# aleflabo/COSKAD

Hardware: AMD Instinct MI355X
Metric: pose_clips_per_sec_fwd_bwd (higher is better)
Workload: dtype f32; 1 GPU; euclidean_encoder_dynamicCenter train step (fwd+mse-to-centre+L2 reg+bwd+Adam), synthetic clips B=4096/GPU T=12 V=17 C=2, channels 2-32-16-32-64, latent 16; clips_per_gpu=4096, global_batch=4096, head=euclidean, parallelism=dp1, hip_graph=False

## Files before the change

### coskad_amd/csrc/fused_apply_bpc.hip

```cpp
#include "fused_ops.h"
#include "layer_launch.h"

namespace coskad {
namespace fpc {

using namespace ff;

#ifndef BPC_GRID
#define BPC_GRID (256 * BPC_OCC)
#endif
#ifndef BPC_OCC
#define BPC_OCC 3
#endif
template <int CT>
__global__ __launch_bounds__(256, BPC_OCC) void k_layer_apply_bpc(const float* __restrict__ in, const float* __restrict__ Zg,
                                                           const float* __restrict__ wfold, const float* __restrict__ bias,
                                                           const float* __restrict__ in_slope, float* __restrict__ out, int B) {
  constexpr int Ci = 16 * CT, Co = 64, CoP = Co, NG = 2 * CT;
  extern __shared__ __attribute__((aligned(16))) float lds[];
  float* r1 = lds;
  float* r2 = lds + 32 * LD;
  const int tid = threadIdx.x, lane = tid & 63;
  const int wave = __builtin_amdgcn_readfirstlane(tid >> 6);
  auto geo = [&]() {
    int l = lane;
    asm volatile("" : "+v"(l));
    return Lane{l & 15, l >> 4};
  };
  Lane L = geo();
  const bool pre = in_slope != nullptr;
  const float a_in = pre ? in_slope[0] : 0.f;
  const BufRes wres = make_res(wfold, 2 * Ci * CoP * 4u);
  const BufRes bres = make_res(bias, CoP * 4u);
  auto clip_res = [&](const float* base, int c, int rows) {
    const bool in_range = c < B;
#ifdef COSKAD_HOT
    return make_res(base + (size_t)(in_range ? (c & 63) : 0) * rows * TV, in_range ? rows * TV * 4u : 0u);
#else
    return make_res(base + (size_t)(in_range ? c : 0) * rows * TV, in_range ? rows * TV * 4u : 0u);
#endif
  };
  constexpr int Q4 = 4 * (TV / 4);
  const bool stg = tid < Q4;
  const int srow = tid / (TV / 4), scol = 4 * (tid - srow * (TV / 4));
  const int svoff = stg ? tid * 16 : 0x7ffffff0;
#ifndef BPC_DEPTH
#define BPC_DEPTH 2
#endif
  constexpr int DEPTH = BPC_DEPTH;
  float4 gq[DEPTH][4];
  auto qload = [&](const BufRes& res, int row0, int q) { return buf_load4(res, svoff, (row0 + 4 * q) * (TV / 4) * 16); };
  auto qstore = [&](int q, float4 v, bool act) {
    if (act) { v.x = prelu(v.x, a_in); v.y = prelu(v.y, a_in); v.z = prelu(v.z, a_in); v.w = prelu(v.w, a_in); }
    if (stg) *reinterpret_cast<float4*>(r2 + (4 * q + srow) * LDW + scol) = v;
  };

  int clip = blockIdx.x;
  {
    const BufRes z0 = clip_res(Zg, clip, Ci), x0 = clip_res(in, clip, Ci);
#pragma unroll
    for (int q = 0; q < 4; ++q) {
      gq[0][q] = qload(z0, 0, q);
      if (DEPTH == 2) gq[DEPTH - 1][q] = CT > 1 ? qload(z0, 16, q) : qload(x0, 0, q);
    }
  }
  for (; clip < B; clip += gridDim.x) {
    const BufRes xres = clip_res(in, clip, Ci), zres = clip_res(Zg, clip, Ci), ores = clip_res(out, clip, Co);
    const BufRes znext = clip_res(Zg, clip + gridDim.x, Ci), xnext = clip_res(in, clip + gridDim.x, Ci);
    auto vload = [&](int vg, int q) {
      const bool nxt = vg >= NG;
      const int g = nxt ? vg - NG : vg;
      return g < CT ? qload(nxt ? znext : zres, 16 * g, q) : qload(nxt ? xnext : xres, 16 * (g - CT), q);
    };
    L = geo();
    const int jc = L.j < T ? L.j : T - 1;
    f32x4 acc[NTILE];
#pragma unroll
    for (int t = 0; t < NTILE; ++t) acc[t] = f32x4{0.f, 0.f, 0.f, 0.f};
#pragma unroll
    for (int q = 0; q < 4; ++q) {
      qstore(q, gq[0][q], false);
      gq[0][q] = vload(DEPTH, q);
    }
    const int lq = (L.q * CoP + 16 * wave + L.j) * 4;
    float wc[2][4];
#pragma unroll
    for (int s = 0; s < 4; ++s) wc[0][s] = buf_load1(wres, lq, (4 * s) * CoP * 4);
    __syncthreads();
#ifndef BPC_BDBL
#define BPC_BDBL 0
#endif
    float b[1 + BPC_BDBL][NTILE];
#pragma unroll
    for (int t = 0; t < NTILE; ++t) b[0][t] = r2[L.q * LDW + (t < T ? t * V + L.j : jc * V + 16)];
#pragma unroll
    for (int g = 0; g < NG; ++g) {
      if (g + 1 < NG) {
#pragma unroll
        for (int s = 0; s < 4; ++s) wc[(g + 1) & 1][s] = buf_load1(wres, lq, ((16 * (g + 1) + 4 * s) * CoP) * 4);
      }
#pragma unroll
      for (int s = 0; s < 4; ++s) {
        if (BPC_BDBL && (s + 1 < 4 || g + 1 < NG)) {
          const int sn = (s + 1) & 3;
#pragma unroll
          for (int t = 0; t < NTILE; ++t) b[(s + 1) & 1][t] = r2[(4 * sn + L.q) * LDW + (t < T ? t * V + L.j : jc * V + 16)];
        }
        if (g + 1 < NG || s == 0) __syncthreads();
        if (g + 1 < NG) {
          qstore(s, gq[(g + 1) % DEPTH][s], g + 1 >= CT && pre);
          if (DEPTH == 2 || g + 2 < NG) gq[(g + 1) % DEPTH][s] = vload(g + 1 + DEPTH, s);
        }
#pragma unroll
        for (int t = 0; t < NTILE; ++t) acc[t] = mfma(wc[g & 1][s], b[BPC_BDBL ? (s & 1) : 0][t], acc[t]);
        if (!BPC_BDBL && (s + 1 < 4 || g + 1 < NG)) {
          const int sn = (s + 1) & 3;
#pragma unroll
          for (int t = 0; t < NTILE; ++t) b[0][t] = r2[(4 * sn + L.q) * LDW + (t < T ? t * V + L.j : jc * V + 16)];
        }
      }
    }
    if (DEPTH == 1) {
#pragma unroll
      for (int q = 0; q < 4; ++q) gq[0][q] = vload(NG, q);
    }
    L = geo();
    const float4 b4 = buf_load4(bres, L.q * 16, (16 * wave) * 4);
    const f32x4 bq = {b4.x, b4.y, b4.z, b4.w};
    const int jf = L.j < T ? L.j : T - 1;
#pragma unroll
    for (int rnd = 0; rnd < 2; ++rnd) {
      if ((wave >> 1) == rnd) {
#pragma unroll
        for (int t = 0; t < NTILE; ++t)
          tile_store(r1, 16 * (wave & 1), t < T ? t * V + L.j : jf * V + 16, t < T || L.j < T, acc[t] + bq, L);
      }
      __syncthreads();
      constexpr int n4 = 32 * (TV / 4);
#pragma unroll
      for (int i = 0; i < (n4 + 255) / 256; ++i) {
        const int e4 = tid + 256 * i;
        const bool ok = e4 < n4;
        const int row = e4 / (TV / 4), col = 4 * (e4 - row * (TV / 4));
        const float* p = r1 + (ok ? row * LD + col : PADCOL);
        const float2 g0 = *reinterpret_cast<const float2*>(p), g1 = *reinterpret_cast<const float2*>(p + 2);
        buf_store4(ores, ok ? e4 * 16 : 0x7ffffff0, (32 * rnd) * (TV / 4) * 16, float4{g0.x, g0.y, g1.x, g1.y});
      }
      __syncthreads();
    }
  }
}

}

int launch_layer_apply_bpc(const float* Z, const float* in, float* out, const float* wfold, const float* bias,
                           const float* in_slope, int B, int Ci, int Co, hipStream_t st) {
  if (!(Ci == 32 && Co == 64)) return fail(COSKAD_ERR_SHAPE, "apply_bpc: built for 32 -> 64 channels (%d, %d)", Ci, Co);
  const size_t lds = (size_t)ff::WAVE_LDS_W * sizeof(float);
  const int grid = B < BPC_GRID ? B : BPC_GRID;
  auto k = fpc::k_layer_apply_bpc<2>;
  {
    ProbeScope probe(KID_LAYER_APPLY, Ci, Co, st);
    hipLaunchKernelGGL(k, dim3(grid), dim3(256), lds, st, in, Z, wfold, bias, in_slope, out, B);
  }
  return check_launch("layer_apply_bpc");
}

}
```

### coskad_amd/csrc/fused_apply_next_bpc.hip

```cpp
#include "fused_ops.h"
#include "layer_launch.h"

namespace coskad {
namespace fnb {

using namespace ff;

#ifndef FNB_OCC
#define FNB_OCC 4
#endif

template <int CT, int OTP>
__global__ __launch_bounds__(256, FNB_OCC) void k_layer_apply_next_bpc(const float* __restrict__ in, const float* __restrict__ Zg,
                                                                      const float* __restrict__ wfold, const float* __restrict__ bias,
                                                                      const float* __restrict__ in_slope,
                                                                      const float* __restrict__ out_slope,
                                                                      const float* __restrict__ ftab, float* __restrict__ out,
                                                                      float* __restrict__ Znext, float* __restrict__ partials, int B) {
  constexpr int Ci = CT ? 16 * CT : 2, Co = 16 * OTP, CoP = Co, NG = 2 * CT;
  constexpr int NACC = OTP == 1 ? 2 : 3;
  constexpr int E = 2 * (Co * Co + Co);
  constexpr int MAXT = OTP == 2 ? 7 : 4;
  extern __shared__ __attribute__((aligned(16))) float lds[];
  float* r1 = lds;
  float* r2 = lds + 32 * LD;
  const int tid = threadIdx.x, lane = tid & 63;
  const int wave = __builtin_amdgcn_readfirstlane(tid >> 6);
  auto geo = [&]() {
    int l = lane;
    asm volatile("" : "+v"(l));
    return Lane{l & 15, l >> 4};
  };
  auto olane = [&]() {
    int l = lane;
    asm volatile("" : "+v"(l));
    return l;
  };
  const bool pre = in_slope != nullptr;
  const float a_in = pre ? in_slope[0] : 0.f;
  const float a_out = out_slope[0];
  const int l16 = lane * 16;
  const BufRes wres = make_res(wfold, 2 * Ci * CoP * 4u);
  const BufRes bres = make_res(bias, CoP * 4u);
  const BufRes tabres = make_res(ftab, LAYER_F4 * 16u);
  auto clip_res = [&](const float* base, int c, int rows) {
    const bool in_range = c < B;
    return make_res(base + (size_t)(in_range ? c : 0) * rows * TV, in_range ? rows * TV * 4u : 0u);
  };
  const int ot = OTP == 2 ? (wave & 1) : 0;
  const int t0 = OTP == 2 ? ((wave >> 1) ? 7 : 0) : (wave == 0 ? 0 : 1 + 3 * wave);
  const int nt = OTP == 2 ? ((wave >> 1) ? 6 : 7) : (wave == 0 ? 4 : 3);
  constexpr int Q4 = 4 * (TV / 4);
  const bool stg = tid < Q4;
  const int srow = tid / (TV / 4), scol = 4 * (tid - srow * (TV / 4));
  const int svoff = stg ? tid * 16 : 0x7ffffff0;
  constexpr int DEPTH = CT == 1 ? 1 : 2;
  float4 gq[DEPTH][4];
  auto qload = [&](const BufRes& res, int row0, int q) { return buf_load4(res, svoff, (row0 + 4 * q) * (TV / 4) * 16); };
  auto qstore = [&](int q, float4 v, bool act) {
    if (act) { v.x = prelu(v.x, a_in); v.y = prelu(v.y, a_in); v.z = prelu(v.z, a_in); v.w = prelu(v.w, a_in); }
    if (stg) *reinterpret_cast<float4*>(r2 + (4 * q + srow) * LDW + scol) = v;
  };
  const bool fst = tid < 2 * (TV / 4);
  const int frow = tid / (TV / 4), fcol = 4 * (tid - frow * (TV / 4));
  const int fvoff = fst ? tid * 16 : 0x7ffffff0;

  f32x4 gx[NACC], gz[NACC];
  float sx[OTP], sz[OTP];
#pragma unroll
  for (int i = 0; i < NACC; ++i) { gx[i] = f32x4{0.f, 0.f, 0.f, 0.f}; gz[i] = f32x4{0.f, 0.f, 0.f, 0.f}; }
#pragma unroll
  for (int i = 0; i < OTP; ++i) { sx[i] = 0.f; sz[i] = 0.f; }
  auto gram_rows = [&](f32x4 (&g)[NACC], float (&s)[OTP], const BufRes& ores, bool act) {
    const Lane L = geo();
    const float* p0 = r1 + L.j * LD + 2 * L.q;
    const float* p1 = r1 + (16 + L.j) * LD + 2 * L.q;
    constexpr int NM = (TV + 7) / 8;
    constexpr int n4 = Co * (TV / 4), NI = (n4 + 63) / 64;
    const int ln = olane();
    for (int m = wave; m < NM; m += 4) {
      float2 a0 = *reinterpret_cast<const float2*>(p0 + 8 * m);
      float2 a1 = OTP == 2 ? *reinterpret_cast<const float2*>(p1 + 8 * m) : float2{0.f, 0.f};
      if (act) {
        a0.x = prelu(a0.x, a_out); a0.y = prelu(a0.y, a_out);
        a1.x = prelu(a1.x, a_out); a1.y = prelu(a1.y, a_out);
      }
      const bool ok = 8 * m + 2 * L.q < TV;
      a0.x = ok ? a0.x : 0.f; a0.y = ok ? a0.y : 0.f;
      a1.x = ok ? a1.x : 0.f; a1.y = ok ? a1.y : 0.f;
      if constexpr (OTP == 1) {
        g[0] = mfma(a0.x, a0.x, g[0]);
        g[1] = mfma(a0.y, a0.y, g[1]);
        s[0] += a0.x + a0.y;
      } else {
        g[0] = mfma(a0.x, a0.x, g[0]);
        g[1] = mfma(a0.x, a1.x, g[1]);
        g[2] = mfma(a1.x, a1.x, g[2]);
        g[0] = mfma(a0.y, a0.y, g[0]);
        g[1] = mfma(a0.y, a1.y, g[1]);
        g[2] = mfma(a1.y, a1.y, g[2]);
        s[0] += a0.x + a0.y;
        s[OTP - 1] += a1.x + a1.y;
      }
      const int i = OTP == 2 ? m : (m & 1 ? -1 : m >> 1);
      if (i >= 0 && i < NI) {
        const int e4 = ln + 64 * i;
        const int row = e4 / (TV / 4), col = 4 * (e4 - row * (TV / 4));
        const bool okp = e4 < n4;
        const float* ptr = r1 + (okp ? row * LD + col : PADCOL);
        const float2 g0 = *reinterpret_cast<const float2*>(ptr), g1 = *reinterpret_cast<const float2*>(ptr + 2);
        buf_store4(ores, okp ? e4 * 16 : 0x7ffffff0, 0, float4{g0.x, g0.y, g1.x, g1.y});
      }
    }
  };

  int clip = blockIdx.x;
  {
    const BufRes z0 = clip_res(Zg, clip, Ci), x0 = clip_res(in, clip, Ci);
    if (CT == 0) {
      gq[0][0] = buf_load4(z0, fvoff, 0);
      gq[0][1] = buf_load4(x0, fvoff, 0);
    } else {
#pragma unroll
      for (int q = 0; q < 4; ++q) {
        gq[0][q] = qload(z0, 0, q);
        if (DEPTH == 2) gq[DEPTH - 1][q] = qload(z0, 16, q);
      }
    }
  }
  for (; clip < B; clip += gridDim.x) {
    const BufRes xres = clip_res(in, clip, Ci), zres = clip_res(Zg, clip, Ci), ores = clip_res(out, clip, Co);
    const BufRes znext = clip_res(Zg, clip + gridDim.x, Ci), xnext = clip_res(in, clip + gridDim.x, Ci);
    const BufRes zores = clip_res(Znext, clip, Co);
    Lane L = geo();
    const int jc = L.j < T ? L.j : T - 1;
    f32x4 acc[MAXT];
#pragma unroll
    for (int t = 0; t < MAXT; ++t) acc[t] = f32x4{0.f, 0.f, 0.f, 0.f};
    auto pos_of = [&](int t) { return t < T ? t * V + L.j : jc * V + 16; };
    const int lq = (L.q * CoP + 16 * ot + L.j) * 4;
    if constexpr (CT == 0) {
      {
        float4 vz = gq[0][0], vx = gq[0][1];
        if (pre) { vx.x = prelu(vx.x, a_in); vx.y = prelu(vx.y, a_in); vx.z = prelu(vx.z, a_in); vx.w = prelu(vx.w, a_in); }
        if (fst) {
          *reinterpret_cast<float4*>(r2 + frow * LDW + fcol) = vz;
          *reinterpret_cast<float4*>(r2 + (2 + frow) * LDW + fcol) = vx;
        }
      }
      const float wc = buf_load1(wres, lq, 0);
      gq[0][0] = buf_load4(znext, fvoff, 0);
      gq[0][1] = buf_load4(xnext, fvoff, 0);
      __syncthreads();
#pragma unroll
      for (int t = 0; t < MAXT; ++t)
        if (t < nt) acc[t] = mfma(wc, r2[L.q * LDW + pos_of(t0 + t)], acc[t]);
    } else {
      auto vload = [&](int vg, int q) {
        const bool nxt = vg >= NG;
        const int g = nxt ? vg - NG : vg;
        return g < CT ? qload(nxt ? znext : zres, 16 * g, q) : qload(nxt ? xnext : xres, 16 * (g - CT), q);
      };
#pragma unroll
      for (int q = 0; q < 4; ++q) {
        qstore(q, gq[0][q], false);
        gq[0][q] = vload(DEPTH, q);
      }
      float wc[2][4];
#pragma unroll
      for (int s = 0; s < 4; ++s) wc[0][s] = buf_load1(wres, lq, (4 * s) * CoP * 4);
      __syncthreads();
      float b[MAXT];
#pragma unroll
      for (int t = 0; t < MAXT; ++t) b[t] = r2[L.q * LDW + pos_of(t0 + (t < nt ? t : 0))];
#pragma unroll
      for (int g = 0; g < NG; ++g) {
        if (g + 1 < NG) {
#pragma unroll
          for (int s = 0; s < 4; ++s) wc[(g + 1) & 1][s] = buf_load1(wres, lq, ((16 * (g + 1) + 4 * s) * CoP) * 4);
        }
#pragma unroll
        for (int s = 0; s < 4; ++s) {
          if (g + 1 < NG || s == 0) __syncthreads();
          if (g + 1 < NG) {
            qstore(s, gq[(g + 1) % DEPTH][s], g + 1 >= CT && pre);
            gq[(g + 1) % DEPTH][s] = vload(g + 1 + DEPTH, s);
          }
#pragma unroll
          for (int t = 0; t < MAXT; ++t)
            if (t < nt) acc[t] = mfma(wc[g & 1][s], b[t], acc[t]);
          if (s + 1 < 4 || g + 1 < NG) {
            const int sn = (s + 1) & 3;
#pragma unroll
            for (int t = 0; t < MAXT; ++t) b[t] = r2[(4 * sn + L.q) * LDW + pos_of(t0 + (t < nt ? t : 0))];
          }
        }
      }
    }
    {
      const float4 b4 = buf_load4(bres, L.q * 16, (16 * ot) * 4);
      const f32x4 bq = {b4.x, b4.y, b4.z, b4.w};
      __syncthreads();
#pragma unroll
      for (int t = 0; t < MAXT; ++t) {
        const int ta = t0 + t;
        if (t < nt) tile_store(r1, 16 * ot, pos_of(ta), ta < T || L.j < T, acc[t] + bq, L);
      }
    }
    __syncthreads();
    gram_rows(gx, sx, ores, true);
    float4 rec = buf_load4(tabres, l16, (wave * 64) * 16);
    __syncthreads();
    L = geo();
    {
      TOp cur[OTP], nxt[OTP];
      f32x4 dprev[OTP];
      int vprev = -1;
#pragma unroll
      for (int rt = 0; rt < OTP; ++rt) cur[rt] = temporal_read<16, true>(r1, rt, wave, L, a_out);
      for (int v = wave; v < V; v += 4) {
        const int vn = v + 4 < V ? v + 4 : v;
        const float4 recn = buf_load4(tabres, l16, (vn * 64) * 16);
#pragma unroll
        for (int rt = 0; rt < OTP; ++rt) nxt[rt] = temporal_read<16, true>(r1, rt, vn, L, a_out);
        f32x4 d[OTP];
#pragma unroll
        for (int rt = 0; rt < OTP; ++rt) d[rt] = temporal_mm(cur[rt], rec);
        if (vprev >= 0) {
#pragma unroll
          for (int rt = 0; rt < OTP; ++rt) temporal_store<16>(r1, rt, vprev, dprev[rt], L);
        }
#pragma unroll
        for (int rt = 0; rt < OTP; ++rt) { dprev[rt] = d[rt]; cur[rt] = nxt[rt]; }
        vprev = v;
        rec = recn;
      }
#pragma unroll
      for (int rt = 0; rt < OTP; ++rt) temporal_store<16>(r1, rt, vprev, dprev[rt], L);
    }
    SpatRec srec = load_spat(tabres, 0, wave, l16);
    __syncthreads();
    L = geo();
    {
      SOp op[OTP];
#pragma unroll
      for (int rt = 0; rt < OTP; ++rt) op[rt] = spatial_read<16>(r1, rt, wave, L);
#pragma unroll
      for (int k = 0; k < T / 4; ++k) {
        const int t = wave + 4 * k, tn = k + 1 < T / 4 ? t + 4 : t;
        const SpatRec nrec = load_spat(tabres, 0, tn, l16);
        SOp opn[OTP];
#pragma unroll
        for (int rt = 0; rt < OTP; ++rt) opn[rt] = spatial_read<16>(r1, rt, tn, L);
#pragma unroll
        for (int rt = 0; rt < OTP; ++rt) {
          const f32x4 d = spatial_mm(op[rt], srec);
          spatial_extra<16>(r1, rt, t, op[rt], srec, L);
          tile_store(r1, 16 * rt, t * V + L.j, true, d, L);
        }
        srec = nrec;
#pragma unroll
        for (int rt = 0; rt < OTP; ++rt) op[rt] = opn[rt];
      }
    }
    __syncthreads();
    gram_rows(gz, sz, zores, false);
  }

  float* row = lds;
  __syncthreads();
  const Lane L = geo();
  auto put = [&](int w, float* base, const f32x4 (&g)[NACC], const float (&s)[OTP]) {
#pragma unroll
    for (int r = 0; r < 4; ++r) {
      const int i = 4 * L.q + r, j = L.j;
      if constexpr (OTP == 1) {
        float* p = base + i * Co + j;
        p[0] = (w ? p[0] : 0.f) + (g[0][r] + g[1][r]);
      } else {
        float* p00 = base + i * Co + j;
        float* p01 = base + i * Co + 16 + j;
        float* p10 = base + (16 + j) * Co + i;
        float* p11 = base + (16 + i) * Co + 16 + j;
        p00[0] = (w ? p00[0] : 0.f) + g[0][r];
        p01[0] = (w ? p01[0] : 0.f) + g[1][r];
        p10[0] = (w ? p10[0] : 0.f) + g[1][r];
        p11[0] = (w ? p11[0] : 0.f) + g[2][r];
      }
// ... 49 lines not shown
```

### coskad_amd/csrc/fused_bwd.hip

```cpp
#include "fused_ops.h"
#include "layer_launch.h"

namespace coskad {
namespace fb {

using namespace ff;

constexpr int PR_A = 0, PR_XA = 12, PR_XB = 13, PR_C = 14, PR_T = 15, PR_N = 32, EROW = PR_N * 256;
constexpr int RE = 32;
__global__ __launch_bounds__(1024) void k_reduce_fused(const float* __restrict__ partials, int P, float* __restrict__ dA,
                                                       float* __restrict__ dT, const float* __restrict__ dap, int ndap,
                                                       float* __restrict__ dslope, int accumulate, const float* __restrict__ brows,
                                                       int bP, int bE, double* __restrict__ bout) {
  __shared__ double sh[1024];
  constexpr int NB = EROW / RE;
  const int col = threadIdx.x % RE;
  if ((int)blockIdx.x > NB) {
    const int e = ((int)blockIdx.x - NB - 1) * RE + col;
    const double t = column_sum_f64<RE>(brows, bP, (size_t)bE, e, e < bE, sh);
    if ((int)threadIdx.x < RE && e < bE) bout[e] = t;
    return;
  }
  if ((int)blockIdx.x == NB) {
    if (!dap) return;
    double s = 0.0;
    for (int i = threadIdx.x; i < ndap; i += 1024) s += (double)dap[i];
    sh[threadIdx.x] = s;
    __syncthreads();
    for (int w = 512; w > 0; w >>= 1) {
      if ((int)threadIdx.x < w) sh[threadIdx.x] += sh[threadIdx.x + w];
      __syncthreads();
    }
    if (threadIdx.x == 0) dslope[0] = accumulate ? dslope[0] + (float)sh[0] : (float)sh[0];
    return;
  }
  const int e = blockIdx.x * RE + col;
  const double t = column_sum_f64<RE>(partials, P, (size_t)EROW, e, true, sh);
  if ((int)threadIdx.x < RE) {
    const int rec = e >> 8, l = (e >> 2) & 63, r = e & 3, j = l & 15, q = l >> 4;
    float* out = nullptr;
    if (rec < PR_XA) out = dA + rec * V * V + (4 * q + r) * V + j;
    else if (rec == PR_XA) { if (4 * q + r < T) out = dA + (4 * q + r) * V * V + 16 * V + j; }
    else if (rec == PR_XB) { if (4 * q + r < T) out = dA + (4 * q + r) * V * V + j * V + 16; }
    else if (rec == PR_C) { if (r == 0 && q == 0 && j < T) out = dA + j * V * V + 16 * V + 16; }
    else if (4 * q + r < T && j < T) out = dT + (rec - PR_T) * T * T + (4 * q + r) * T + j;
    if (out) *out = accumulate ? *out + (float)t : (float)t;
  }
}

constexpr int bpc_occ(int CT, int NS) { return CT == 1 && NS == 0 ? 3 : 2; }
#ifndef FBB_BDBL
#define FBB_BDBL 0
#endif
#ifndef FBB_SKIP
#define FBB_SKIP 0
#endif

template <int CT, int OT, int NS, int CB>
__global__ __launch_bounds__(256, bpc_occ(CT, NS)) void k_layer_bwd_bpc(const float* __restrict__ in, const float* __restrict__ Zg,
                                                               const float* __restrict__ dU, const float* __restrict__ coef,
                                                               const float* __restrict__ btab, const float* __restrict__ in_slope,
                                                               float* __restrict__ dIn, float* __restrict__ partials,
                                                               float* __restrict__ dap, int B, const float* __restrict__ below_z,
                                                               const float* __restrict__ below_x, const float* __restrict__ below_slope,
                                                               float* __restrict__ below_stats) {
  constexpr int Ci = 16 * CT, Co = 16 * OT, CiP = Ci, NG = OT + CT;
  constexpr int KT0 = (Co + Ci) * CiP, DX0 = KT0 + CiP, KR0 = DX0 + (Co + Ci) * CiP;
  constexpr int MAXF = CT == 2 ? 6 : 3;
  extern __shared__ __attribute__((aligned(16))) float lds[];
  float* r1 = lds;
  float* r2 = lds + 32 * LD;
  float* zs = lds + WAVE_LDS_W + 256 * (threadIdx.x >> 6);
  const int tid = threadIdx.x, lane = tid & 63;
  const int wave = __builtin_amdgcn_readfirstlane(tid >> 6);
  auto geo = [&]() {
    int l = lane;
    asm volatile("" : "+v"(l));
    return Lane{l & 15, l >> 4};
  };
  Lane L = geo();
  const float a_in = in_slope[0];
  const int l16 = lane * 16;
  const BufRes tabres = make_res(btab, BTAB_F4 * 16u);
  const BufRes cres = make_res(coef, (KR0 + CiP) * 4u);
  auto clip_res = [&](const float* base, int c, int rows) {
    const bool in_range = c < B;
#ifdef COSKAD_HOT
    return make_res(base + (size_t)(in_range ? (c & 63) : 0) * rows * TV, in_range ? rows * TV * 4u : 0u);
#else
    return make_res(base + (size_t)(in_range ? c : 0) * rows * TV, in_range ? rows * TV * 4u : 0u);
#endif
  };
  const int ct = CT == 2 ? (wave & 1) : 0;
  const int f0 = CT == 2 ? 6 * (wave >> 1) : 3 * wave;
  const bool owns16 = CT == 2 ? (wave >> 1) == 1 : wave == 3;
  constexpr int Q4 = 4 * (TV / 4);
  const bool stg = tid < Q4;
  const int srow = tid / (TV / 4), scol = 4 * (tid - srow * (TV / 4));
  const int svoff = stg ? tid * 16 : 0x7ffffff0;
  auto qload = [&](const BufRes& res, int row0, int q) { return buf_load4(res, svoff, (row0 + 4 * q) * (TV / 4) * 16); };
  auto qstore = [&](int q, float4 v, bool act, float slope, int stride) {
    if (act) { v.x = prelu(v.x, slope); v.y = prelu(v.y, slope); v.z = prelu(v.z, slope); v.w = prelu(v.w, slope); }
    *reinterpret_cast<float2*>(r2 + (stg ? (4 * q + srow) * stride + scol : 15 * stride + PADCOL)) = float2{v.x, v.y};
    *reinterpret_cast<float2*>(r2 + (stg ? (4 * q + srow) * stride + scol + 2 : 15 * stride + PADCOL)) = float2{v.z, v.w};
  };
  constexpr int N4 = Ci * (TV / 4), XL = (N4 + 255) / 256;
  float4 xs[XL];
  auto xload = [&](float4 (&dst)[XL], const BufRes& r) {
#pragma unroll
    for (int i = 0; i < XL; ++i) dst[i] = buf_load4(r, (tid + 256 * i) < N4 ? (tid + 256 * i) * 16 : 0x7ffffff0, 0);
  };
  f32x4 dAacc[MAXF], exA = {0.f, 0.f, 0.f, 0.f}, exB = {0.f, 0.f, 0.f, 0.f};
  constexpr int MAXJ = (V + 3) / 4;
  f32x4 dTacc[MAXJ];
  float corner = 0.f, da = 0.f;
#pragma unroll
  for (int t = 0; t < MAXF; ++t) dAacc[t] = f32x4{0.f, 0.f, 0.f, 0.f};
#pragma unroll
  for (int k = 0; k < MAXJ; ++k) dTacc[k] = f32x4{0.f, 0.f, 0.f, 0.f};
  constexpr int NGB = NS == 2 ? 2 * CB : 1;
  f32x4 nsb[NGB][CT];
  float nss[CT];
#pragma unroll
  for (int g = 0; g < NGB; ++g)
#pragma unroll
    for (int c = 0; c < CT; ++c) nsb[g][c] = f32x4{0.f, 0.f, 0.f, 0.f};
#pragma unroll
  for (int c = 0; c < CT; ++c) nss[c] = 0.f;
  const bool bpre = NS != 0 && below_slope != nullptr;
  const float a_b = bpre ? below_slope[0] : 0.f;

  auto temporal_rr = [&](int base4) {
    const Lane Lt = geo();
    TOp cur[CT], nxt[CT];
    f32x4 dprev[CT];
    int vprev = -1;
#pragma unroll
    for (int rt = 0; rt < CT; ++rt) cur[rt] = temporal_read<16>(r1, rt, wave, Lt);
    float4 rec = buf_load4(tabres, l16, (base4 + wave * 64) * 16);
    for (int v = wave; v < V; v += 4) {
      const int vn = v + 4 < V ? v + 4 : v;
      const float4 recn = buf_load4(tabres, l16, (base4 + vn * 64) * 16);
#pragma unroll
      for (int rt = 0; rt < CT; ++rt) nxt[rt] = temporal_read<16>(r1, rt, vn, Lt);
      f32x4 d[CT];
#pragma unroll
      for (int rt = 0; rt < CT; ++rt) d[rt] = temporal_mm(cur[rt], rec);
      if (vprev >= 0) {
#pragma unroll
        for (int rt = 0; rt < CT; ++rt) temporal_store<16>(r1, rt, vprev, dprev[rt], Lt);
      }
#pragma unroll
      for (int rt = 0; rt < CT; ++rt) { dprev[rt] = d[rt]; cur[rt] = nxt[rt]; }
      vprev = v;
      rec = recn;
    }
#pragma unroll
    for (int rt = 0; rt < CT; ++rt) temporal_store<16>(r1, rt, vprev, dprev[rt], Lt);
  };
  auto spatial_rr = [&]() {
    const Lane Ls = geo();
    SpatRec srec = load_spat(tabres, 0, wave, l16);
    SOp op[CT];
#pragma unroll
    for (int rt = 0; rt < CT; ++rt) op[rt] = spatial_read<16>(r1, rt, wave, Ls);
#pragma unroll
    for (int k = 0; k < T / 4; ++k) {
      const int t = wave + 4 * k, tn = k + 1 < T / 4 ? t + 4 : t;
      const SpatRec nrec = load_spat(tabres, 0, tn, l16);
      SOp opn[CT];
#pragma unroll
      for (int rt = 0; rt < CT; ++rt) opn[rt] = spatial_read<16>(r1, rt, tn, Ls);
#pragma unroll
      for (int rt = 0; rt < CT; ++rt) {
        const f32x4 d = spatial_mm(op[rt], srec);
        spatial_extra<16>(r1, rt, t, op[rt], srec, Ls);
        tile_store(r1, 16 * rt, t * V + Ls.j, true, d, Ls);
      }
      srec = nrec;
#pragma unroll
      for (int rt = 0; rt < CT; ++rt) op[rt] = opn[rt];
    }
  };

  int clip = blockIdx.x;
  float4 gq[4];
  {
    xload(xs, clip_res(in, clip, Ci));
    const BufRes du0 = clip_res(dU, clip, Co);
#pragma unroll
    for (int q = 0; q < 4; ++q) gq[q] = qload(du0, 0, q);
  }
  for (; clip < B; clip += gridDim.x) {
    const BufRes xres = clip_res(in, clip, Ci), zres = clip_res(Zg, clip, Ci), dures = clip_res(dU, clip, Co);
    const BufRes ores = clip_res(dIn, clip, Ci);
    auto kload = [&](int g, int q, const BufRes& res2) { return g < OT ? qload(dures, 16 * g, q) : qload(res2, 16 * (g - OT), q); };
    __syncthreads();
#pragma unroll
    for (int i = 0; i < XL; ++i) {
      const int e4 = tid + 256 * i;
      float4 v = xs[i];
      v.x = prelu(v.x, a_in); v.y = prelu(v.y, a_in); v.z = prelu(v.z, a_in); v.w = prelu(v.w, a_in);
      const int row = e4 / (TV / 4), col = 4 * (e4 - row * (TV / 4));
      *reinterpret_cast<float2*>(r1 + (e4 < N4 ? row * LD + col : PADCOL)) = float2{v.x, v.y};
      *reinterpret_cast<float2*>(r1 + (e4 < N4 ? row * LD + col + 2 : PADCOL)) = float2{v.z, v.w};
    }
#pragma unroll
    for (int q = 0; q < 4; ++q) {
      qstore(q, gq[q], false, 0.f, LDW);
      gq[q] = kload(1, q, zres);
    }
    __syncthreads();
    if (!(FBB_SKIP & 1)) temporal_rr(0);
    L = geo();
    const int lq = (L.q * CiP + 16 * ct + L.j) * 4;
    const int jc = L.j < T ? L.j : T - 1;
    auto pos_of = [&](int k) { return k < MAXF ? (f0 + k) * V + L.j : jc * V + 16; };
    auto kpass = [&](f32x4 (&acc)[MAXF + 1], f32x4 (&acc2)[MAXF + 1], const BufRes& res2, bool act2, int c0, int c1, int c2,
                     bool with16, bool with16b) {
      constexpr bool DUAL = true;
      float wc[2][4], wc2[2][4];
      auto cload = [&](int buf, int g) {
        const int krow = g < OT ? c0 + 16 * g : c1 + 16 * (g - OT);
#pragma unroll
        for (int s = 0; s < 4; ++s) {
          wc[buf][s] = buf_load1(cres, lq, ((krow + 4 * s) * CiP) * 4);
          if (DUAL && g < OT) wc2[buf][s] = buf_load1(cres, lq, ((c2 + 16 * g + 4 * s) * CiP) * 4);
        }
      };
      cload(0, 0);
      float b[1 + FBB_BDBL][MAXF + 1];
#pragma unroll
      for (int k = 0; k <= MAXF; ++k) b[0][k] = r2[L.q * LDW + pos_of(k)];
#pragma unroll
      for (int g = 0; g < NG; ++g) {
        if (g + 1 < NG) cload((g + 1) & 1, g + 1);
#pragma unroll
        for (int s = 0; s < 4; ++s) {
          if (g + 1 < NG || s == 0) __syncthreads();
          const int sn = (s + 1) & 3;
          if (FBB_BDBL && (s + 1 < 4 || g + 1 < NG)) {
            __builtin_amdgcn_sched_barrier(0);
#pragma unroll
            for (int k = 0; k <= MAXF; ++k) b[(s + 1) & 1][k] = r2[(4 * sn + L.q) * LDW + pos_of(k)];
            __builtin_amdgcn_sched_barrier(0);
          }
          if (g + 1 < NG) {
            qstore(s, gq[s], g + 1 >= OT && act2, a_in, LDW);
            if (g + 2 < NG) gq[s] = kload(g + 2, s, res2);
          }
#pragma unroll
          for (int k = 0; k <= MAXF; ++k)
            if (k < MAXF || with16) acc[k] = mfma(wc[g & 1][s], b[FBB_BDBL ? (s & 1) : 0][k], acc[k]);
          if (DUAL && g < OT) {
#pragma unroll
            for (int k = 0; k <= MAXF; ++k)
              if (k < MAXF || with16b) acc2[k] = mfma(wc2[g & 1][s], b[FBB_BDBL ? (s & 1) : 0][k], acc2[k]);
          }
          if (!FBB_BDBL && (s + 1 < 4 || g + 1 < NG)) {
#pragma unroll
            for (int k = 0; k <= MAXF; ++k) b[0][k] = r2[(4 * sn + L.q) * LDW + pos_of(k)];
          }
        }
      }
    };
    f32x4 az[MAXF + 1];
    {
      const float4 a = buf_load4(cres, L.q * 16, (KT0 + 16 * ct) * 4);
#pragma unroll
      for (int k = 0; k <= MAXF; ++k) az[k] = f32x4{a.x, a.y, a.z, a.w};
    }
    f32x4 xr[MAXF + 1];
    {
      const float4 kq = buf_load4(cres, L.q * 16, (KR0 + 16 * ct) * 4);
#pragma unroll
      for (int k = 0; k <= MAXF; ++k) xr[k] = f32x4{kq.x, kq.y, kq.z, kq.w};
    }
    __syncthreads();
    if (!(FBB_SKIP & 2)) kpass(az, xr, zres, false, 0, Co, DX0 / CiP, true, owns16);
#pragma unroll
    for (int q = 0; q < 4; ++q) gq[q] = qload(xres, 0, q);
    if (owns16) {
      const f32x4 y16 = tile_load(r1, 16 * ct, jc * V + 16, L);
#pragma unroll
      for (int r = 0; r < 4; ++r) corner = fmaf(y16[r], az[MAXF][r], corner);
    }
    *reinterpret_cast<f32x4*>(zs + lane * 4) = az[MAXF];
#pragma unroll
    for (int k = 0; k < ((FBB_SKIP & 4) ? 0 : MAXF); ++k) {
      const int t = f0 + k;
      const f32x4 y = tile_load(r1, 16 * ct, t * V + L.j, L);
      const f32x4 y16 = tile_load(r1, 16 * ct, t * V + 16, L);
      const f32x4 dz16 = *reinterpret_cast<const f32x4*>(zs + (16 * L.q + t) * 4);
      float pa = 0.f, pb = 0.f;
#pragma unroll
      for (int r = 0; r < 4; ++r) {
        dAacc[k] = mfma(y[r], az[k][r], dAacc[k]);
        pa = fmaf(y16[r], az[k][r], pa);
        pb = fmaf(y[r], dz16[r], pb);
      }
      const float sel = L.j == t ? 1.f : 0.f;
      exA = mfma(sel, pa, exA);
      exB = mfma(sel, pb, exB);
    }
    __syncthreads();
#pragma unroll
    for (int k = 0; k < MAXF; ++k) tile_store(r1, 16 * ct, (f0 + k) * V + L.j, true, az[k], L);
    if (owns16) tile_store(r1, 16 * ct, jc * V + 16, L.j < T, az[MAXF], L);
    __syncthreads();
    if (!(FBB_SKIP & 8)) spatial_rr();
    __syncthreads();
    L = geo();
    {
      const int ic = L.j < T ? L.j : T - 1;
#pragma unroll
      for (int h = 0; h < ((FBB_SKIP & 16) ? 0 : CT); ++h) {
#pragma unroll
        for (int q = 0; q < 4; ++q) {
          qstore(q, gq[q], true, a_in, LDW);
          if (h + 1 < CT) gq[q] = qload(xres, 16 * (h + 1), q);
        }
        float wk[4];
#pragma unroll
        for (int s = 0; s < 4; ++s) wk[s] = buf_load1(cres, lq, ((DX0 / CiP + Co + 16 * h + 4 * s) * CiP) * 4);
        __syncthreads();
#pragma unroll
        for (int s = 0; s < 4; ++s) {
          if (!(FBB_SKIP & 2)) {
            float bx[MAXF + 1];
#pragma unroll
            for (int k = 0; k <= MAXF; ++k) bx[k] = r2[(4 * s + L.q) * LDW + pos_of(k)];
#pragma unroll
            for (int k = 0; k <= MAXF; ++k)
              if (k < MAXF || owns16) xr[k] = mfma(wk[s], bx[k], xr[k]);
          }
#pragma unroll
          for (int k = 0; k < MAXJ; ++k) {
            const int v = wave + 4 * k;
            if (v < V) {
              const float a = r2[(4 * s + L.q) * LDW + ic * V + v];
              const float bb = r1[(16 * h + 4 * s + L.q) * LD + ic * V + v];
              dTacc[k] = mfma(L.j < T ? a : 0.f, L.j < T ? bb : 0.f, dTacc[k]);
            }
          }
        }
        __syncthreads();
      }
    }
    float4 u[XL];
    {
      if (!(FBB_SKIP & 1)) temporal_rr(TEMP_F4 + SPAT_F4);
      __syncthreads();
      xload(u, xres);
      L = geo();
#pragma unroll
      for (int k = 0; k < MAXF; ++k) {
        const int pos = (f0 + k) * V + L.j;
        tile_store(r1, 16 * ct, pos, true, xr[k] + tile_load(r1, 16 * ct, pos, L), L);
      }
      if (owns16) {
        const int pos = (L.j < T ? L.j : T - 1) * V + 16;
        tile_store(r1, 16 * ct, pos, L.j < T, xr[MAXF] + tile_load(r1, 16 * ct, pos, L), L);
      }
    }
    __syncthreads();
    if (!(FBB_SKIP & 32)) {
      const BufRes xn = clip_res(in, clip + gridDim.x, Ci), dun = clip_res(dU, clip + gridDim.x, Co);
      float4 pg[4];
      if constexpr (NS == 1) {
        const int fv = tid < 2 * (TV / 4) ? tid * 16 : 0x7ffffff0;
        pg[0] = buf_load4(clip_res(below_z, clip, 2), fv, 0);
        pg[1] = buf_load4(clip_res(below_x, clip, 2), fv, 0);
      }
      if constexpr (NS == 2) {
#pragma unroll
        for (int q = 0; q < 4; ++q) gq[q] = qload(clip_res(below_z, clip, 16 * CB), 0, q);
      } else {
#pragma unroll
        for (int q = 0; q < 4; ++q) gq[q] = qload(dun, 0, q);
      }
#pragma unroll
      for (int i = 0; i < XL; ++i) {
        const int e4 = tid + 256 * i;
        const int row = e4 / (TV / 4), col = 4 * (e4 - row * (TV / 4));
        float* p = r1 + (e4 < N4 ? row * LD + col : PADCOL);
        float* p2 = r1 + (e4 < N4 ? row * LD + col + 2 : PADCOL);
        const float2 g0 = *reinterpret_cast<const float2*>(p), g1 = *reinterpret_cast<const float2*>(p2);
        float g[4] = {g0.x, g0.y, g1.x, g1.y};
        if (e4 < N4) {
          const float uu[4] = {u[i].x, u[i].y, u[i].z, u[i].w};
#pragma unroll
          for (int c = 0; c < 4; ++c) {
            if (uu[c] < 0.f) da = fmaf(g[c], uu[c], da);
            g[c] = uu[c] > 0.f ? g[c] : a_in * g[c];
          }
        }
        buf_store4(ores, e4 < N4 ? e4 * 16 : 0x7ffffff0, 0, float4{g[0], g[1], g[2], g[3]});
        if constexpr (NS != 0) {
          *reinterpret_cast<float2*>(p) = float2{g[0], g[1]};
          *reinterpret_cast<float2*>(p2) = float2{g[2], g[3]};
        }
      }
      xload(xs, xn);
      if constexpr (NS == 1) {
// ... 87 lines not shown
#pragma unroll
      for (int k = 0; k < MAXJ; ++k)
        if (wave + 4 * k < V) add4(PR_T + wave + 4 * k, dTacc[k]);
      if (lane == 0) extra[0] += da;
      if constexpr (NS == 1) {
#pragma unroll
        for (int c = 0; c < CT; ++c) {
#pragma unroll
          for (int r = 0; r < 4; ++r) {
            const int o = 16 * c + 4 * L.q + r;
            if (L.j < 4) extra[64 + (L.j < 2 ? o * 2 + L.j : 2 * Ci + o * 2 + (L.j - 2))] += nsb[0][c][r];
          }
          const float t = quad_sum(nss[c]);
          if (L.q == 0) extra[64 + 4 * Ci + 16 * c + L.j] += t;
        }
      }
      if constexpr (NS == 2) {
#pragma unroll
        for (int g = 0; g < NGB; ++g)
#pragma unroll
          for (int c = 0; c < CT; ++c)
#pragma unroll
            for (int r = 0; r < 4; ++r) {
              const int o = 16 * c + 4 * L.q + r;
              extra[64 + (g < CB ? 0 : Ci * Cb) + o * Cb + 16 * (g < CB ? g : g - CB) + L.j] += nsb[g][c][r];
            }
#pragma unroll
        for (int c = 0; c < CT; ++c) {
          const float t = quad_sum(nss[c]);
          if (L.q == 0) extra[64 + 2 * Ci * Cb + 16 * c + L.j] += t;
        }
      }
    }
    __syncthreads();
  }
  float4* prow = reinterpret_cast<float4*>(partials + (size_t)blockIdx.x * EROW);
  for (int e = tid; e < PR_N * 64; e += 256) prow[e] = row4[e];
  if (tid == 0 && dap) dap[blockIdx.x] = extra[0];
  if constexpr (NS != 0) {
    for (int e = tid; e < NSE; e += 256) below_stats[(size_t)blockIdx.x * NSE + e] = extra[64 + e];
  }
}

}

int bwd_bpc_rows(int B, int Ci, bool chain) {
  const int grid = 256 * fb::bpc_occ(Ci / 16, chain ? 1 : 0);
  return B < grid ? B : grid;
}

int launch_layer_bwd_bpc(const float* in, const float* Zg, const float* dU, const float* coef, const float* in_slope, float* dIn,
                         float* btab, float* partials, float* dap, int B, int Ci, int Co, hipStream_t st, int* rows_out,
                         const float* below_z, const float* below_x, const float* below_slope, int below_Ci, float* below_stats) {
  const size_t lds = (size_t)(ff::WAVE_LDS_W + 4 * 256) * sizeof(float);
  const int grid = bwd_bpc_rows(B, Ci, below_stats != nullptr);
  *rows_out = grid;
#define LAUNCH_FBB(CT, OT, NS, CB)                                                                                   \
  do {                                                                                                               \
    auto k = fb::k_layer_bwd_bpc<CT, OT, NS, CB>;                                                                   \
    hipLaunchKernelGGL(k, dim3(grid), dim3(256), lds, st, in, Zg, dU, coef, btab, in_slope, dIn, partials, dap, B,   \
                       below_z, below_x, below_slope, below_stats);                                                  \
  } while (0)
  {
    ProbeScope probe(KID_BWD_DATA, Ci, Co, st);
    if (below_stats) {
      if (Ci == 32 && Co == 16 && below_Ci == 2) LAUNCH_FBB(2, 1, 1, 0);
      else if (Ci == 16 && Co == 32 && below_Ci == 32) LAUNCH_FBB(1, 2, 2, 2);
      else if (Ci == 32 && Co == 64 && below_Ci == 16) LAUNCH_FBB(2, 4, 2, 1);
      else return fail(COSKAD_ERR_SHAPE, "bwd_bpc: no kernel forms the reductions of a %d-channel layer below (%d -> %d)", below_Ci, Ci, Co);
    } else if (Ci == 16 && Co == 16) LAUNCH_FBB(1, 1, 0, 0);
    else if (Ci == 16 && Co == 32) LAUNCH_FBB(1, 2, 0, 0);
    else if (Ci == 16 && Co == 64) LAUNCH_FBB(1, 4, 0, 0);
    else if (Ci == 32 && Co == 16) LAUNCH_FBB(2, 1, 0, 0);
    else if (Ci == 32 && Co == 32) LAUNCH_FBB(2, 2, 0, 0);
    else if (Ci == 32 && Co == 64) LAUNCH_FBB(2, 4, 0, 0);
    else return fail(COSKAD_ERR_SHAPE, "bwd_bpc: unsupported channels (%d, %d)", Ci, Co);
  }
#undef LAUNCH_FBB
  return check_launch("bwd_bpc");
}

int launch_reduce_fused(const float* partials, int rows, float* dA, float* dT, const float* dap, float* dslope, int accumulate,
                        hipStream_t st, const float* brows, int bE, double* bout) {
  const int extra = brows ? 1 + ceil_div(bE, fb::RE) : (dap ? 1 : 0);
  hipLaunchKernelGGL(fb::k_reduce_fused, dim3(fb::EROW / fb::RE + extra), dim3(1024), 0, st, partials, rows, dA, dT, dap, rows,
                     dslope, accumulate, brows, rows, bE, bout);
  return check_launch("bwd_reduce_fused");
}

int layer_bwd_below_rows(int T_, int V_, int B, int Ci, int Co, int below_Ci) {
  const bool built = (Ci == 32 && Co == 16 && below_Ci == 2) || (Ci == 16 && Co == 32 && below_Ci == 32) ||
                     (Ci == 32 && Co == 64 && below_Ci == 16);
  if (!(T_ == ff::T && V_ == ff::V && built) || B <= 0) return 0;
  return bwd_bpc_rows(B, Ci, true);
}

bool layer_bwd_fused_ok(int T_, int V_, int Ci, int Co) {
  return T_ == ff::T && V_ == ff::V && (Ci == 16 || Ci == 32) && (Co == 16 || Co == 32 || Co == 64);
}

}
```

Before: 3.052 million clips/s.

## Hoist per-layer weights out of clip loops and stage backward tables in LDS

Result: faster. 3.111 million clips/s, median of 6 (+1.9%).

```diff
diff --git a/coskad_amd/csrc/fused_apply_bpc.hip b/coskad_amd/csrc/fused_apply_bpc.hip
--- a/coskad_amd/csrc/fused_apply_bpc.hip
+++ b/coskad_amd/csrc/fused_apply_bpc.hip
@@ -55,6 +55,15 @@
     if (stg) *reinterpret_cast<float4*>(r2 + (4 * q + srow) * LDW + scol) = v;
   };
 
+  const int lq = (L.q * CoP + 16 * wave + L.j) * 4;
+  const float4 b4 = buf_load4(bres, L.q * 16, (16 * wave) * 4);
+  const f32x4 bq = {b4.x, b4.y, b4.z, b4.w};
+  float wc[NG][4];
+#pragma unroll
+  for (int g = 0; g < NG; ++g)
+#pragma unroll
+    for (int s = 0; s < 4; ++s) wc[g][s] = buf_load1(wres, lq, ((16 * g + 4 * s) * CoP) * 4);
+
   int clip = blockIdx.x;
   {
     const BufRes z0 = clip_res(Zg, clip, Ci), x0 = clip_res(in, clip, Ci);
@@ -82,10 +91,6 @@
       qstore(q, gq[0][q], false);
       gq[0][q] = vload(DEPTH, q);
     }
-    const int lq = (L.q * CoP + 16 * wave + L.j) * 4;
-    float wc[2][4];
-#pragma unroll
-    for (int s = 0; s < 4; ++s) wc[0][s] = buf_load1(wres, lq, (4 * s) * CoP * 4);
     __syncthreads();
 #ifndef BPC_BDBL
 #define BPC_BDBL 0
@@ -95,10 +100,6 @@
     for (int t = 0; t < NTILE; ++t) b[0][t] = r2[L.q * LDW + (t < T ? t * V + L.j : jc * V + 16)];
 #pragma unroll
     for (int g = 0; g < NG; ++g) {
-      if (g + 1 < NG) {
-#pragma unroll
-        for (int s = 0; s < 4; ++s) wc[(g + 1) & 1][s] = buf_load1(wres, lq, ((16 * (g + 1) + 4 * s) * CoP) * 4);
-      }
 #pragma unroll
       for (int s = 0; s < 4; ++s) {
         if (BPC_BDBL && (s + 1 < 4 || g + 1 < NG)) {
@@ -112,7 +113,7 @@
           if (DEPTH == 2 || g + 2 < NG) gq[(g + 1) % DEPTH][s] = vload(g + 1 + DEPTH, s);
         }
 #pragma unroll
-        for (int t = 0; t < NTILE; ++t) acc[t] = mfma(wc[g & 1][s], b[BPC_BDBL ? (s & 1) : 0][t], acc[t]);
+        for (int t = 0; t < NTILE; ++t) acc[t] = mfma(wc[g][s], b[BPC_BDBL ? (s & 1) : 0][t], acc[t]);
         if (!BPC_BDBL && (s + 1 < 4 || g + 1 < NG)) {
           const int sn = (s + 1) & 3;
 #pragma unroll
@@ -125,8 +126,6 @@
       for (int q = 0; q < 4; ++q) gq[0][q] = vload(NG, q);
     }
     L = geo();
-    const float4 b4 = buf_load4(bres, L.q * 16, (16 * wave) * 4);
-    const f32x4 bq = {b4.x, b4.y, b4.z, b4.w};
     const int jf = L.j < T ? L.j : T - 1;
 #pragma unroll
     for (int rnd = 0; rnd < 2; ++rnd) {
diff --git a/coskad_amd/csrc/fused_apply_next_bpc.hip b/coskad_amd/csrc/fused_apply_next_bpc.hip
--- a/coskad_amd/csrc/fused_apply_next_bpc.hip
+++ b/coskad_amd/csrc/fused_apply_next_bpc.hip
@@ -21,6 +21,7 @@
   constexpr int NACC = OTP == 1 ? 2 : 3;
   constexpr int E = 2 * (Co * Co + Co);
   constexpr int MAXT = OTP == 2 ? 7 : 4;
+  constexpr bool TREC_HOIST = CT == 0;
   extern __shared__ __attribute__((aligned(16))) float lds[];
   float* r1 = lds;
   float* r2 = lds + 32 * LD;
@@ -114,6 +115,28 @@
     }
   };
 
+  const Lane Lp = geo();
+  const int lq = (Lp.q * CoP + 16 * ot + Lp.j) * 4;
+  const float4 b4 = buf_load4(bres, Lp.q * 16, (16 * ot) * 4);
+  const f32x4 bq = {b4.x, b4.y, b4.z, b4.w};
+  constexpr int NWC = CT ? NG : 1;
+  float wc[NWC][4];
+  if constexpr (CT == 0) {
+    wc[0][0] = buf_load1(wres, lq, 0);
+  } else {
+#pragma unroll
+    for (int g = 0; g < NG; ++g)
+#pragma unroll
+      for (int s = 0; s < 4; ++s) wc[g][s] = buf_load1(wres, lq, ((16 * g + 4 * s) * CoP) * 4);
+  }
+  constexpr int NTR = (V + 3) / 4;
+  float4 trec[NTR];
+  auto load_trec = [&]() {
+#pragma unroll
+    for (int i = 0; i < NTR; ++i) trec[i] = buf_load4(tabres, l16, ((wave + 4 * i < V ? wave + 4 * i : wave) * 64) * 16);
+  };
+  if constexpr (TREC_HOIST) load_trec();
+
   int clip = blockIdx.x;
   {
     const BufRes z0 = clip_res(Zg, clip, Ci), x0 = clip_res(in, clip, Ci);
@@ -138,7 +161,6 @@
 #pragma unroll
     for (int t = 0; t < MAXT; ++t) acc[t] = f32x4{0.f, 0.f, 0.f, 0.f};
     auto pos_of = [&](int t) { return t < T ? t * V + L.j : jc * V + 16; };
-    const int lq = (L.q * CoP + 16 * ot + L.j) * 4;
     if constexpr (CT == 0) {
       {
         float4 vz = gq[0][0], vx = gq[0][1];
@@ -148,13 +170,12 @@
           *reinterpret_cast<float4*>(r2 + (2 + frow) * LDW + fcol) = vx;
         }
       }
-      const float wc = buf_load1(wres, lq, 0);
       gq[0][0] = buf_load4(znext, fvoff, 0);
       gq[0][1] = buf_load4(xnext, fvoff, 0);
       __syncthreads();
 #pragma unroll
       for (int t = 0; t < MAXT; ++t)
-        if (t < nt) acc[t] = mfma(wc, r2[L.q * LDW + pos_of(t0 + t)], acc[t]);
+        if (t < nt) acc[t] = mfma(wc[0][0], r2[L.q * LDW + pos_of(t0 + t)], acc[t]);
     } else {
       auto vload = [&](int vg, int q) {
         const bool nxt = vg >= NG;
@@ -166,19 +187,12 @@
         qstore(q, gq[0][q], false);
         gq[0][q] = vload(DEPTH, q);
       }
-      float wc[2][4];
-#pragma unroll
-      for (int s = 0; s < 4; ++s) wc[0][s] = buf_load1(wres, lq, (4 * s) * CoP * 4);
       __syncthreads();
       float b[MAXT];
 #pragma unroll
       for (int t = 0; t < MAXT; ++t) b[t] = r2[L.q * LDW + pos_of(t0 + (t < nt ? t : 0))];
 #pragma unroll
       for (int g = 0; g < NG; ++g) {
-        if (g + 1 < NG) {
-#pragma unroll
-          for (int s = 0; s < 4; ++s) wc[(g + 1) & 1][s] = buf_load1(wres, lq, ((16 * (g + 1) + 4 * s) * CoP) * 4);
-        }
 #pragma unroll
         for (int s = 0; s < 4; ++s) {
           if (g + 1 < NG || s == 0) __syncthreads();
@@ -188,7 +202,7 @@
           }
 #pragma unroll
           for (int t = 0; t < MAXT; ++t)
-            if (t < nt) acc[t] = mfma(wc[g & 1][s], b[t], acc[t]);
+            if (t < nt) acc[t] = mfma(wc[g][s], b[t], acc[t]);
           if (s + 1 < 4 || g + 1 < NG) {
             const int sn = (s + 1) & 3;
 #pragma unroll
@@ -198,8 +212,6 @@
       }
     }
     {
-      const float4 b4 = buf_load4(bres, L.q * 16, (16 * ot) * 4);
-      const f32x4 bq = {b4.x, b4.y, b4.z, b4.w};
       __syncthreads();
 #pragma unroll
       for (int t = 0; t < MAXT; ++t) {
@@ -208,8 +220,8 @@
       }
     }
     __syncthreads();
+    if constexpr (!TREC_HOIST) load_trec();
     gram_rows(gx, sx, ores, true);
-    float4 rec = buf_load4(tabres, l16, (wave * 64) * 16);
     __syncthreads();
     L = geo();
     {
@@ -218,22 +230,24 @@
       int vprev = -1;
 #pragma unroll
       for (int rt = 0; rt < OTP; ++rt) cur[rt] = temporal_read<16, true>(r1, rt, wave, L, a_out);
-      for (int v = wave; v < V; v += 4) {
-        const int vn = v + 4 < V ? v + 4 : v;
-        const float4 recn = buf_load4(tabres, l16, (vn * 64) * 16);
-#pragma unroll
-        for (int rt = 0; rt < OTP; ++rt) nxt[rt] = temporal_read<16, true>(r1, rt, vn, L, a_out);
-        f32x4 d[OTP];
-#pragma unroll
-        for (int rt = 0; rt < OTP; ++rt) d[rt] = temporal_mm(cur[rt], rec);
-        if (vprev >= 0) {
-#pragma unroll
-          for (int rt = 0; rt < OTP; ++rt) temporal_store<16>(r1, rt, vprev, dprev[rt], L);
+#pragma unroll
+      for (int i = 0; i < NTR; ++i) {
+        const int v = wave + 4 * i;
+        if (v < V) {
+          const int vn = v + 4 < V ? v + 4 : v;
+#pragma unroll
+          for (int rt = 0; rt < OTP; ++rt) nxt[rt] = temporal_read<16, true>(r1, rt, vn, L, a_out);
+          f32x4 d[OTP];
+#pragma unroll
+          for (int rt = 0; rt < OTP; ++rt) d[rt] = temporal_mm(cur[rt], trec[i]);
+          if (i > 0) {
+#pragma unroll
+            for (int rt = 0; rt < OTP; ++rt) temporal_store<16>(r1, rt, vprev, dprev[rt], L);
+          }
+#pragma unroll
+          for (int rt = 0; rt < OTP; ++rt) { dprev[rt] = d[rt]; cur[rt] = nxt[rt]; }
+          vprev = v;
         }
-#pragma unroll
-        for (int rt = 0; rt < OTP; ++rt) { dprev[rt] = d[rt]; cur[rt] = nxt[rt]; }
-        vprev = v;
-        rec = recn;
       }
 #pragma unroll
       for (int rt = 0; rt < OTP; ++rt) temporal_store<16>(r1, rt, vprev, dprev[rt], L);
diff --git a/coskad_amd/csrc/fused_bwd.hip b/coskad_amd/csrc/fused_bwd.hip
--- a/coskad_amd/csrc/fused_bwd.hip
+++ b/coskad_amd/csrc/fused_bwd.hip
@@ -49,6 +49,11 @@
 }
 
 constexpr int bpc_occ(int CT, int NS) { return CT == 1 && NS == 0 ? 3 : 2; }
+constexpr bool bpc_tlds(int CT, int OT, int NS) { return bpc_occ(CT, NS) == 2 && OT < 4; }
+constexpr int TF_F = V * 3 * 64, AS_F = T * 5 * 64, ET_F = 256;
+constexpr int bpc_lds_floats(int CT, int OT, int NS) {
+  return WAVE_LDS_W + 4 * 256 + (bpc_tlds(CT, OT, NS) ? TF_F + AS_F + ET_F + CT * CT * 256 + 2 * 16 * CT : 0);
+}
 #ifndef FBB_BDBL
 #define FBB_BDBL 0
 #endif
@@ -71,6 +76,12 @@
   float* r1 = lds;
   float* r2 = lds + 32 * LD;
   float* zs = lds + WAVE_LDS_W + 256 * (threadIdx.x >> 6);
+  constexpr bool TLDS = bpc_tlds(CT, OT, NS);
+  float* tf = lds + WAVE_LDS_W + 4 * 256;
+  float* as = tf + TF_F;
+  float* et = as + AS_F;
+  float* krl = et + ET_F;
+  float* kql = krl + CT * CT * 256;
   const int tid = threadIdx.x, lane = tid & 63;
   const int wave = __builtin_amdgcn_readfirstlane(tid >> 6);
   auto geo = [&]() {
@@ -130,17 +141,25 @@
   const bool bpre = NS != 0 && below_slope != nullptr;
   const float a_b = bpre ? below_slope[0] : 0.f;
 
-  auto temporal_rr = [&](int base4) {
+  auto temporal_rr = [&](int base4, auto from_lds) {
     const Lane Lt = geo();
+    auto trec = [&](int v) {
+      if constexpr (decltype(from_lds)::value) {
+        const float* p = tf + v * 192 + 16 * Lt.q + Lt.j;
+        return float4{p[0], p[64], p[128], 0.f};
+      } else {
+        return buf_load4(tabres, l16, (base4 + v * 64) * 16);
+      }
+    };
     TOp cur[CT], nxt[CT];
     f32x4 dprev[CT];
     int vprev = -1;
 #pragma unroll
     for (int rt = 0; rt < CT; ++rt) cur[rt] = temporal_read<16>(r1, rt, wave, Lt);
-    float4 rec = buf_load4(tabres, l16, (base4 + wave * 64) * 16);
+    float4 rec = trec(wave);
     for (int v = wave; v < V; v += 4) {
       const int vn = v + 4 < V ? v + 4 : v;
-      const float4 recn = buf_load4(tabres, l16, (base4 + vn * 64) * 16);
+      const float4 recn = trec(vn);
 #pragma unroll
       for (int rt = 0; rt < CT; ++rt) nxt[rt] = temporal_read<16>(r1, rt, vn, Lt);
       f32x4 d[CT];
@@ -160,14 +179,23 @@
   };
   auto spatial_rr = [&]() {
     const Lane Ls = geo();
-    SpatRec srec = load_spat(tabres, 0, wave, l16);
+    auto spat_rec = [&](int t) {
+      if constexpr (TLDS) {
+        const float* p = as + t * 320 + 16 * Ls.q + Ls.j;
+        const float* e = et + t * 20 + Ls.q;
+        return SpatRec{float4{p[0], p[64], p[128], p[192]}, float4{p[256], e[0], e[4], e[8]}, float4{e[12], e[16], 0.f, 0.f}};
+      } else {
+        return load_spat(tabres, 0, t, l16);
+      }
+    };
+    SpatRec srec = spat_rec(wave);
     SOp op[CT];
 #pragma unroll
     for (int rt = 0; rt < CT; ++rt) op[rt] = spatial_read<16>(r1, rt, wave, Ls);
 #pragma unroll
     for (int k = 0; k < T / 4; ++k) {
       const int t = wave + 4 * k, tn = k + 1 < T / 4 ? t + 4 : t;
-      const SpatRec nrec = load_spat(tabres, 0, tn, l16);
+      const SpatRec nrec = spat_rec(tn);
       SOp opn[CT];
 #pragma unroll
       for (int rt = 0; rt < CT; ++rt) opn[rt] = spatial_read<16>(r1, rt, tn, Ls);
@@ -183,6 +211,28 @@
     }
   };
 
+  auto stage_params = [&]() {
+    for (int e = tid; e < V * 64; e += 256) {
+      const float4 r = buf_load4(tabres, e * 16, 0);
+      float* p = tf + (e >> 6) * 192 + (e & 63);
+      p[0] = r.x; p[64] = r.y; p[128] = r.z;
+    }
+    for (int e = tid; e < T * 64; e += 256) {
+      const int t = e >> 6, l = e & 63, o = (TEMP_F4 + t * 3 * 64 + l) * 16;
+      const float4 c0 = buf_load4(tabres, o, 0), c1 = buf_load4(tabres, o, 1024), c2 = buf_load4(tabres, o, 2048);
+      float* p = as + t * 320 + l;
+      p[0] = c0.x; p[64] = c0.y; p[128] = c0.z; p[192] = c0.w; p[256] = c1.x;
+      if ((l & 15) == 0) {
+        float* q = et + t * 20 + (l >> 4);
+        q[0] = c1.y; q[4] = c1.z; q[8] = c1.w; q[12] = c2.x; q[16] = c2.y;
+      }
+    }
+    for (int e = tid; e < CT * CT * 256; e += 256) {
+      const int l = e & 63, c = (e >> 6) % CT, hs = (e >> 6) / CT;
+      krl[e] = buf_load1(cres, ((DX0 / CiP + Co + 4 * hs + (l >> 4)) * CiP + 16 * c + (l & 15)) * 4, 0);
+    }
+    if (tid < 2 * Ci) kql[tid] = buf_load1(cres, ((tid < Ci ? KT0 : KR0 - Ci) + tid) * 4, 0);
+  };
   int clip = blockIdx.x;
   float4 gq[4];
   {
@@ -191,6 +241,7 @@
 #pragma unroll
     for (int q = 0; q < 4; ++q) gq[q] = qload(du0, 0, q);
   }
+  if constexpr (TLDS) stage_params();
   for (; clip < B; clip += gridDim.x) {
     const BufRes xres = clip_res(in, clip, Ci), zres = clip_res(Zg, clip, Ci), dures = clip_res(dU, clip, Co);
     const BufRes ores = clip_res(dIn, clip, Ci);
@@ -211,7 +262,7 @@
       gq[q] = kload(1, q, zres);
     }
     __syncthreads();
-    if (!(FBB_SKIP & 1)) temporal_rr(0);
+    if (!(FBB_SKIP & 1)) temporal_rr(0, std::integral_constant<bool, TLDS>{});
     L = geo();
     const int lq = (L.q * CiP + 16 * ct + L.j) * 4;
     const int jc = L.j < T ? L.j : T - 1;
@@ -266,13 +317,13 @@
     };
     f32x4 az[MAXF + 1];
     {
-      const float4 a = buf_load4(cres, L.q * 16, (KT0 + 16 * ct) * 4);
+      const float4 a = TLDS ? *reinterpret_cast<const float4*>(kql + 16 * ct + 4 * L.q) : buf_load4(cres, L.q * 16, (KT0 + 16 * ct) * 4);
 #pragma unroll
       for (int k = 0; k <= MAXF; ++k) az[k] = f32x4{a.x, a.y, a.z, a.w};
     }
     f32x4 xr[MAXF + 1];
     {
-      const float4 kq = buf_load4(cres, L.q * 16, (KR0 + 16 * ct) * 4);
+      const float4 kq = TLDS ? *reinterpret_cast<const float4*>(kql + Ci + 16 * ct + 4 * L.q) : buf_load4(cres, L.q * 16, (KR0 + 16 * ct) * 4);
 #pragma unroll
       for (int k = 0; k <= MAXF; ++k) xr[k] = f32x4{kq.x, kq.y, kq.z, kq.w};
     }
@@ -322,7 +373,8 @@
         }
         float wk[4];
 #pragma unroll
-        for (int s = 0; s < 4; ++s) wk[s] = buf_load1(cres, lq, ((DX0 / CiP + Co + 16 * h + 4 * s) * CiP) * 4);
+        for (int s = 0; s < 4; ++s)
+          wk[s] = TLDS ? krl[((4 * h + s) * CT + ct) * 64 + 16 * L.q + L.j] : buf_load1(cres, lq, ((DX0 / CiP + Co + 16 * h + 4 * s) * CiP) * 4);
         __syncthreads();
 #pragma unroll
         for (int s = 0; s < 4; ++s) {
@@ -349,7 +401,7 @@
     }
     float4 u[XL];
     {
-      if (!(FBB_SKIP & 1)) temporal_rr(TEMP_F4 + SPAT_F4);
+      if (!(FBB_SKIP & 1)) temporal_rr(TEMP_F4 + SPAT_F4, std::false_type{});
       __syncthreads();
       xload(u, xres);
       L = geo();
@@ -543,15 +595,16 @@
 int launch_layer_bwd_bpc(const float* in, const float* Zg, const float* dU, const float* coef, const float* in_slope, float* dIn,
                          float* btab, float* partials, float* dap, int B, int Ci, int Co, hipStream_t st, int* rows_out,
                          const float* below_z, const float* below_x, const float* below_slope, int below_Ci, float* below_stats) {
-  const size_t lds = (size_t)(ff::WAVE_LDS_W + 4 * 256) * sizeof(float);
   const int grid = bwd_bpc_rows(B, Ci, below_stats != nullptr);
   *rows_out = grid;
 #define LAUNCH_FBB(CT, OT, NS, CB)                                                                                   \
   do {                                                                                                               \
-    auto k = fb::k_layer_bwd_bpc<CT, OT, NS, CB>;                                                                   \
-    hipLaunchKernelGGL(k, dim3(grid), dim3(256), lds, st, in, Zg, dU, coef, btab, in_slope, dIn, partials, dap, B,   \
-                       below_z, below_x, below_slope, below_stats);                                                  \
+    rc = launch_lds<fb::k_layer_bwd_bpc<CT, OT, NS, CB>>("bwd_bpc", dim3(grid), dim3(256),                          \
+                                                         fb::bpc_lds_floats(CT, OT, NS) * sizeof(float), st, in, Zg, dU, coef,  \
+                                                         (const float*)btab, in_slope, dIn, partials, dap, B, below_z,      \
+                                                         below_x, below_slope, below_stats);                                \
   } while (0)
+  int rc = COSKAD_OK;
   {
     ProbeScope probe(KID_BWD_DATA, Ci, Co, st);
     if (below_stats) {
@@ -568,7 +621,7 @@
     else return fail(COSKAD_ERR_SHAPE, "bwd_bpc: unsupported channels (%d, %d)", Ci, Co);
   }
 #undef LAUNCH_FBB
-  return check_launch("bwd_bpc");
+  return rc;
 }
 
 int launch_reduce_fused(const float* partials, int rows, float* dA, float* dT, const float* dap, float* dslope, int accumulate,
```
